# Gadersd/stable-diffusion-xl-burn

Hardware: NVIDIA H100
Metric: unet_sampler_steps_per_sec_1024x1024_bs1 (higher is better)
Workload: dtype f16

## Files before the change

stable-diffusion-xl-burn_b200/csrc/attention.cu:

```cuda
#include <stdlib.h>

#include "common.cuh"
#include "kernels.h"

namespace sdxl {

static constexpr int kTileBytes = 128 * 128;
static constexpr int kKvStages = 3;
static constexpr int kConsumerWarps = 8;
static constexpr int kAttnThreads = kConsumerWarps * 32 + 32;
static constexpr int kAttnSmem = 1024  + kTileBytes + 2 * kKvStages * kTileBytes + 256;

__device__ __forceinline__ float ex2_approx(float x) {
  float y;
  asm("ex2.approx.ftz.f32 %0, %1;" : "=f"(y) : "f"(x));
  return y;
}
__device__ __forceinline__ uint32_t pack_half2(float a, float b) {
  __half2 t = __floats2half2_rn(a, b);
  return *reinterpret_cast<uint32_t*>(&t);
}

__device__ __forceinline__ void attn_key_block(float (&o)[32], float (&m)[2], float (&l)[2], uint32_t q_addr, const uint8_t* sK,
                                               const uint8_t* sV, uint64_t* kv_full, uint64_t* kv_empty, int j, int kb, int S,
                                               float sl2e, int lane) {
  const int st = j % kKvStages;
  mbar_wait_nocall(&kv_full[st], (j / kKvStages) & 1);
  float s[64];
  wg_fence();
  const uint32_t k_addr = smem_u32(sK + st * kTileBytes);
#pragma unroll
  for (int k = 0; k < 4; ++k) wgmma_ss_n128(s, wg_desc_sw128(q_addr + 32 * k), wg_desc_sw128(k_addr + 32 * k), k);
  wg_commit();
  wg_wait<0>();
  if (kb * 128 + 128 > S) {
#pragma unroll
    for (int jj = 0; jj < 16; ++jj)
#pragma unroll
      for (int e = 0; e < 2; ++e)
        if (kb * 128 + 8 * jj + 2 * (lane & 3) + e >= S) { s[4 * jj + e] = -INFINITY; s[4 * jj + 2 + e] = -INFINITY; }
  }
  uint32_t pa[32];
#pragma unroll
  for (int h = 0; h < 2; ++h) {
    float mx = -INFINITY;
#pragma unroll
    for (int jj = 0; jj < 16; ++jj) mx = fmaxf(mx, fmaxf(s[4 * jj + 2 * h], s[4 * jj + 2 * h + 1]));
    mx = fmaxf(mx, __shfl_xor_sync(0xffffffffu, mx, 1));
    mx = fmaxf(mx, __shfl_xor_sync(0xffffffffu, mx, 2));
    const float m_new = fmaxf(m[h], mx);
    const float alpha = ex2_approx((m[h] - m_new) * sl2e);
    const float mb = m_new * sl2e;
    float sum = 0.f;
#pragma unroll
    for (int jj = 0; jj < 16; ++jj) {
      const float p0 = ex2_approx(fmaf(s[4 * jj + 2 * h], sl2e, -mb));
      const float p1 = ex2_approx(fmaf(s[4 * jj + 2 * h + 1], sl2e, -mb));
      sum += p0 + p1;
      pa[4 * (jj >> 1) + 2 * (jj & 1) + h] = pack_half2(p0, p1);
    }
    l[h] = l[h] * alpha + sum;
    m[h] = m_new;
#pragma unroll
    for (int jj = 0; jj < 8; ++jj) { o[4 * jj + 2 * h] *= alpha; o[4 * jj + 2 * h + 1] *= alpha; }
  }
  wg_fence();
  const uint32_t v_addr = smem_u32(sV + st * kTileBytes);
#pragma unroll
  for (int kk = 0; kk < 8; ++kk)
    wgmma_rs_n64_tb(o, *reinterpret_cast<const uint32_t(*)[4]>(pa + 4 * kk), wg_desc_sw128(v_addr + 2048 * kk));
  wg_commit();
  wg_wait<0>();
  if (lane == 0) mbar_arrive(&kv_empty[st]);
}

template <bool kIp>
__global__ void __launch_bounds__(kAttnThreads, 1) attention_kernel(const __grid_constant__ AttnParams p) {
  extern __shared__ uint8_t smem_raw[];
  uint8_t* smem = reinterpret_cast<uint8_t*>((reinterpret_cast<uintptr_t>(smem_raw) + 1023) & ~uintptr_t(1023));
  uint8_t* sQ = smem;
  uint8_t* sK = sQ + kTileBytes;
  uint8_t* sV = sK + kKvStages * kTileBytes;
  uint64_t* bars = reinterpret_cast<uint64_t*>(sV + kKvStages * kTileBytes);
  uint64_t* q_full = bars;
  uint64_t* kv_full = q_full + 1;
  uint64_t* kv_empty = kv_full + kKvStages;

  const int warp = threadIdx.x >> 5, lane = threadIdx.x & 31;
  const int nblk = (p.S + 127) / 128;
  const int nqt = (p.T + 127) / 128;
  const int qt = blockIdx.x % nqt, head = (blockIdx.x / nqt) % p.n_head, b = blockIdx.x / (nqt * p.n_head);

  if (threadIdx.x == 0) {
    tma_prefetch_desc(&p.tmQ);
    tma_prefetch_desc(&p.tmK);
    tma_prefetch_desc(&p.tmV);
    if constexpr (kIp) {
      tma_prefetch_desc(&p.tmKip);
      tma_prefetch_desc(&p.tmVip);
    }
    mbar_init(q_full, 1);
    for (int i = 0; i < kKvStages; ++i) { mbar_init(&kv_full[i], 1); mbar_init(&kv_empty[i], kConsumerWarps); }
    fence_barrier_init();
  }
  __syncthreads();
  griddep_wait();
  griddep_launch_dependents();

  if (warp == kConsumerWarps) {
    if (lane != 0) return;
    mbar_expect_tx(q_full, kTileBytes);
    tma_load_3d(sQ, &p.tmQ, q_full, p.q_col0 + head * 64, qt * 128, b);
    for (int j = 0; j < nblk; ++j) {
      const int st = j % kKvStages;
      mbar_wait_nocall(&kv_empty[st], ((j / kKvStages) & 1) ^ 1);
      mbar_expect_tx(&kv_full[st], 2 * kTileBytes);
      tma_load_3d(sK + st * kTileBytes, &p.tmK, &kv_full[st], p.k_col0 + head * 64, j * 128, b);
      tma_load_3d(sV + st * kTileBytes, &p.tmV, &kv_full[st], p.v_col0 + head * 64, j * 128, b);
    }
    if constexpr (kIp) {
      const int nblk_ip = (p.S_ip + 127) / 128;
      for (int j = nblk; j < nblk + nblk_ip; ++j) {
        const int st = j % kKvStages;
        mbar_wait_nocall(&kv_empty[st], ((j / kKvStages) & 1) ^ 1);
        mbar_expect_tx(&kv_full[st], 2 * kTileBytes);
        tma_load_3d(sK + st * kTileBytes, &p.tmKip, &kv_full[st], p.k_ip_col0 + head * 64, (j - nblk) * 128, b);
        tma_load_3d(sV + st * kTileBytes, &p.tmVip, &kv_full[st], p.v_ip_col0 + head * 64, (j - nblk) * 128, b);
      }
    }
    return;
  }

  const int wg = warp >> 2;
  const float sl2e = p.scale_log2e;
  const uint32_t q_addr = smem_u32(sQ) + (uint32_t)wg * (64 * 128);
  float o[32];
#pragma unroll
  for (int i = 0; i < 32; ++i) o[i] = 0.f;
  float m[2] = {-INFINITY, -INFINITY}, l[2] = {0.f, 0.f};
  mbar_wait_nocall(q_full, 0);
  for (int j = 0; j < nblk; ++j) {
    const int st = j % kKvStages;
    mbar_wait_nocall(&kv_full[st], (j / kKvStages) & 1);
    float s[64];
    wg_fence();
    const uint32_t k_addr = smem_u32(sK + st * kTileBytes);
#pragma unroll
    for (int k = 0; k < 4; ++k) wgmma_ss_n128(s, wg_desc_sw128(q_addr + 32 * k), wg_desc_sw128(k_addr + 32 * k), k);
    wg_commit();
    wg_wait<0>();
    if (j * 128 + 128 > p.S) {
#pragma unroll
      for (int jj = 0; jj < 16; ++jj)
#pragma unroll
        for (int e = 0; e < 2; ++e)
          if (j * 128 + 8 * jj + 2 * (lane & 3) + e >= p.S) { s[4 * jj + e] = -INFINITY; s[4 * jj + 2 + e] = -INFINITY; }
    }
    uint32_t pa[32];
#pragma unroll
    for (int h = 0; h < 2; ++h) {
      float mx = -INFINITY;
#pragma unroll
      for (int jj = 0; jj < 16; ++jj) mx = fmaxf(mx, fmaxf(s[4 * jj + 2 * h], s[4 * jj + 2 * h + 1]));
      mx = fmaxf(mx, __shfl_xor_sync(0xffffffffu, mx, 1));
      mx = fmaxf(mx, __shfl_xor_sync(0xffffffffu, mx, 2));
      const float m_new = fmaxf(m[h], mx);
      const float alpha = ex2_approx((m[h] - m_new) * sl2e);
      const float mb = m_new * sl2e;
      float sum = 0.f;
#pragma unroll
      for (int jj = 0; jj < 16; ++jj) {
        const float p0 = ex2_approx(fmaf(s[4 * jj + 2 * h], sl2e, -mb));
        const float p1 = ex2_approx(fmaf(s[4 * jj + 2 * h + 1], sl2e, -mb));
        sum += p0 + p1;
        pa[4 * (jj >> 1) + 2 * (jj & 1) + h] = pack_half2(p0, p1);
      }
      l[h] = l[h] * alpha + sum;
      m[h] = m_new;
#pragma unroll
      for (int jj = 0; jj < 8; ++jj) { o[4 * jj + 2 * h] *= alpha; o[4 * jj + 2 * h + 1] *= alpha; }
    }
    wg_fence();
    const uint32_t v_addr = smem_u32(sV + st * kTileBytes);
#pragma unroll
    for (int kk = 0; kk < 8; ++kk)
      wgmma_rs_n64_tb(o, *reinterpret_cast<const uint32_t(*)[4]>(pa + 4 * kk), wg_desc_sw128(v_addr + 2048 * kk));
    wg_commit();
    wg_wait<0>();
    if (lane == 0) mbar_arrive(&kv_empty[st]);
  }
  float ot[kIp ? 32 : 1];
  float s_ip = 0.f;
  if constexpr (kIp) {
#pragma unroll
    for (int h = 0; h < 2; ++h) {
      float lt = l[h];
      lt += __shfl_xor_sync(0xffffffffu, lt, 1);
      lt += __shfl_xor_sync(0xffffffffu, lt, 2);
      const float inv = 1.0f / lt;
#pragma unroll
      for (int jj = 0; jj < 8; ++jj) {
        ot[4 * jj + 2 * h] = o[4 * jj + 2 * h] * inv;
        ot[4 * jj + 2 * h + 1] = o[4 * jj + 2 * h + 1] * inv;
      }
      m[h] = -INFINITY;
      l[h] = 0.f;
    }
#pragma unroll
    for (int i = 0; i < 32; ++i) o[i] = 0.f;
    const int nblk_ip = (p.S_ip + 127) / 128;
    for (int j = nblk; j < nblk + nblk_ip; ++j) attn_key_block(o, m, l, q_addr, sK, sV, kv_full, kv_empty, j, j - nblk, p.S_ip, sl2e, lane);
    s_ip = *p.ip_scale;
  }
  const int r = wg * 64 + (warp & 3) * 16 + (lane >> 2);
#pragma unroll
  for (int h = 0; h < 2; ++h) {
    float lt = l[h];
    lt += __shfl_xor_sync(0xffffffffu, lt, 1);
    lt += __shfl_xor_sync(0xffffffffu, lt, 2);
    const float inv = 1.0f / lt;
    const int t = qt * 128 + r + 8 * h;
    if (t < p.T) {
      __half* out = p.out + ((size_t)b * p.T + t) * p.ldo + head * 64 + 2 * (lane & 3);
#pragma unroll
      for (int jj = 0; jj < 8; ++jj) {
        if constexpr (kIp)
          *reinterpret_cast<__half2*>(out + 8 * jj) = __floats2half2_rn(fmaf(s_ip, o[4 * jj + 2 * h] * inv, ot[4 * jj + 2 * h]),
                                                                        fmaf(s_ip, o[4 * jj + 2 * h + 1] * inv, ot[4 * jj + 2 * h + 1]));
        else
          *reinterpret_cast<__half2*>(out + 8 * jj) = __floats2half2_rn(o[4 * jj + 2 * h] * inv, o[4 * jj + 2 * h + 1] * inv);
      }
    }
  }
}

static bool g_attn_attr[2][64];
int attention_launch(cudaStream_t st, const AttnParams& p) {
  if (p.T < 1 || p.S < 1 || (p.ldo & 1)) return 2002;
  const bool ip = p.S_ip > 0;
  if (ip && !p.ip_scale) return 2002;
  auto kernel = ip ? attention_kernel<true> : attention_kernel<false>;
  int r = smem_optin(kernel, kAttnSmem, g_attn_attr[ip]);
  if (r) return r;
  const long tiles = (long)p.B * p.n_head * ((p.T + 127) / 128);
  return launch_kernel(kernel, dim3((unsigned)tiles), dim3(kAttnThreads), (size_t)kAttnSmem, st, true, p);
}

}
```

stable-diffusion-xl-burn_b200/csrc/common.cuh:

```cuda
#pragma once
#include <cuda_fp16.h>
#include <cuda_runtime.h>
#include <stdint.h>
#include <stdio.h>

namespace sdxl {

__device__ __forceinline__ uint32_t smem_u32(const void* p) {
  return static_cast<uint32_t>(__cvta_generic_to_shared(p));
}
__device__ __forceinline__ float warp_sum(float v) {
#pragma unroll
  for (int o = 16; o > 0; o >>= 1) v += __shfl_xor_sync(0xffffffffu, v, o);
  return v;
}
__device__ __forceinline__ float warp_max(float v) {
#pragma unroll
  for (int o = 16; o > 0; o >>= 1) v = fmaxf(v, __shfl_xor_sync(0xffffffffu, v, o));
  return v;
}
__device__ __forceinline__ float silu_f(float x) { return x / (1.0f + __expf(-x)); }
__device__ __forceinline__ float erf_as(float x) {
  const float ax = fabsf(x);
  float t;
  asm("rcp.approx.ftz.f32 %0, %1;" : "=f"(t) : "f"(fmaf(0.3275911f, ax, 1.0f)));
  const float poly =
      t * (0.254829592f + t * (-0.284496736f + t * (1.421413741f + t * (-1.453152027f + t * 1.061405429f))));
  float e;
  asm("ex2.approx.ftz.f32 %0, %1;" : "=f"(e) : "f"(-ax * ax * 1.4426950408889634f));
  return copysignf(1.0f - poly * e, x);
}
__device__ __forceinline__ float gelu_erf_f(float x) {
  return 0.5f * x * (1.0f + erf_as(x * 0.70710678118654752440f));
}
__device__ __forceinline__ uint64_t globaltimer_ns() {
  uint64_t t;
  asm volatile("mov.u64 %0, %globaltimer;" : "=l"(t)::"memory");
  return t;
}

template <int N>
__device__ __forceinline__ void setmaxnreg_dec() { asm volatile("setmaxnreg.dec.sync.aligned.u32 %0;" ::"n"(N)); }
template <int N>
__device__ __forceinline__ void setmaxnreg_inc() { asm volatile("setmaxnreg.inc.sync.aligned.u32 %0;" ::"n"(N)); }

__device__ __forceinline__ void griddep_wait() { asm volatile("griddepcontrol.wait;" ::: "memory"); }
__device__ __forceinline__ void griddep_launch_dependents() {
  asm volatile("griddepcontrol.launch_dependents;" ::: "memory");
}

__device__ __forceinline__ void mbar_init(uint64_t* bar, uint32_t count) {
  asm volatile("mbarrier.init.shared::cta.b64 [%0], %1;" ::"r"(smem_u32(bar)), "r"(count));
}
__device__ __forceinline__ void fence_barrier_init() {
  asm volatile("fence.mbarrier_init.release.cluster;" ::: "memory");
}
__device__ __forceinline__ void mbar_expect_tx(uint64_t* bar, uint32_t bytes) {
  asm volatile("mbarrier.arrive.expect_tx.shared::cta.b64 _, [%0], %1;" ::"r"(smem_u32(bar)),
               "r"(bytes)
               : "memory");
}
__device__ __forceinline__ void mbar_arrive(uint64_t* bar) {
  asm volatile("mbarrier.arrive.shared::cta.b64 _, [%0];" ::"r"(smem_u32(bar)) : "memory");
}
__device__ __forceinline__ bool mbar_try_wait(uint64_t* bar, uint32_t parity) {
  uint32_t ok;
  asm volatile(
      "{\n\t"
      ".reg .pred p;\n\t"
      "mbarrier.try_wait.parity.shared::cta.b64 p, [%1], %2;\n\t"
      "selp.u32 %0, 1, 0, p;\n\t"
      "}"
      : "=r"(ok)
      : "r"(smem_u32(bar)), "r"(parity)
      : "memory");
  return ok != 0;
}
__device__ __forceinline__ void mbar_wait(uint64_t* bar, uint32_t parity) {
  if (mbar_try_wait(bar, parity)) return;
  const uint64_t t0 = globaltimer_ns();
  while (!mbar_try_wait(bar, parity)) {
    if (globaltimer_ns() - t0 > 4000000000ull) {
      printf("sdxl_b200: mbarrier wait timeout (block %d,%d,%d thread %d)\n", blockIdx.x, blockIdx.y,
             blockIdx.z, threadIdx.x);
      __trap();
    }
  }
}
__device__ __forceinline__ void mbar_wait_nocall(uint64_t* bar, uint32_t parity) {
  if (mbar_try_wait(bar, parity)) return;
  const uint64_t t0 = globaltimer_ns();
  while (!mbar_try_wait(bar, parity))
    if (globaltimer_ns() - t0 > 4000000000ull) __trap();
}
__device__ __forceinline__ void fence_proxy_async_smem() {
  asm volatile("fence.proxy.async.shared::cta;" ::: "memory");
}

__device__ __forceinline__ void tma_prefetch_desc(const void* tmap) {
  asm volatile("prefetch.tensormap [%0];" ::"l"(reinterpret_cast<uint64_t>(tmap)) : "memory");
}
__device__ __forceinline__ void tma_load_2d(void* dst, const void* tmap, uint64_t* bar, int c0, int c1) {
  asm volatile(
      "cp.async.bulk.tensor.2d.shared::cluster.global.mbarrier::complete_tx::bytes [%0], [%1, {%3, %4}], [%2];"
      ::"r"(smem_u32(dst)), "l"(reinterpret_cast<uint64_t>(tmap)), "r"(smem_u32(bar)), "r"(c0), "r"(c1)
      : "memory");
}
__device__ __forceinline__ void tma_load_3d(void* dst, const void* tmap, uint64_t* bar, int c0, int c1,
                                            int c2) {
  asm volatile(
      "cp.async.bulk.tensor.3d.shared::cluster.global.mbarrier::complete_tx::bytes [%0], [%1, {%3, %4, %5}], [%2];"
      ::"r"(smem_u32(dst)), "l"(reinterpret_cast<uint64_t>(tmap)), "r"(smem_u32(bar)), "r"(c0), "r"(c1),
      "r"(c2)
      : "memory");
}
__device__ __forceinline__ void tma_load_4d(void* dst, const void* tmap, uint64_t* bar, int c0, int c1,
                                            int c2, int c3) {
  asm volatile(
      "cp.async.bulk.tensor.4d.shared::cluster.global.mbarrier::complete_tx::bytes [%0], [%1, {%3, %4, %5, %6}], [%2];"
      ::"r"(smem_u32(dst)), "l"(reinterpret_cast<uint64_t>(tmap)), "r"(smem_u32(bar)), "r"(c0), "r"(c1),
      "r"(c2), "r"(c3)
      : "memory");
}

__device__ __forceinline__ void wg_fence() { asm volatile("wgmma.fence.sync.aligned;" ::: "memory"); }
__device__ __forceinline__ void wg_commit() { asm volatile("wgmma.commit_group.sync.aligned;" ::: "memory"); }
template <int N>
__device__ __forceinline__ void wg_wait() {
  asm volatile("wgmma.wait_group.sync.aligned %0;" ::"n"(N) : "memory");
}
__device__ __forceinline__ uint64_t wg_desc_sw128(uint32_t saddr) {
  const uint32_t lo = ((saddr >> 4) & 0x3FFFu) | (1u << 16);
  const uint32_t hi = 64u  | (1u << 30) ;
  return (static_cast<uint64_t>(hi) << 32) | lo;
}
__device__ __forceinline__ void wgmma_ss_n160(float (&d)[80], uint64_t da, uint64_t db, int scale_d) {
  asm volatile(
      "{\n\t.reg .pred p;\n\tsetp.ne.b32 p, %82, 0;\n\t"
      "wgmma.mma_async.sync.aligned.m64n160k16.f32.f16.f16 {%0, %1, %2, %3, %4, %5, %6, %7, %8, %9, %10, %11, %12, %13, %14, %15, %16, %17, %18, %19, %20, %21, %22, %23, %24, %25, %26, %27, %28, %29, %30, %31, %32, %33, %34, %35, %36, %37, %38, %39, %40, %41, %42, %43, %44, %45, %46, %47, %48, %49, %50, %51, %52, %53, %54, %55, %56, %57, %58, %59, %60, %61, %62, %63, %64, %65, %66, %67, %68, %69, %70, %71, %72, %73, %74, %75, %76, %77, %78, %79}, %80, %81, p, 1, 1, 0, 0;\n\t}"
      : "+f"(d[0]), "+f"(d[1]), "+f"(d[2]), "+f"(d[3]), "+f"(d[4]), "+f"(d[5]), "+f"(d[6]), "+f"(d[7]), "+f"(d[8]), "+f"(d[9]), "+f"(d[10]), "+f"(d[11]), "+f"(d[12]), "+f"(d[13]), "+f"(d[14]), "+f"(d[15]), "+f"(d[16]), "+f"(d[17]), "+f"(d[18]), "+f"(d[19]), "+f"(d[20]), "+f"(d[21]), "+f"(d[22]), "+f"(d[23]), "+f"(d[24]), "+f"(d[25]), "+f"(d[26]), "+f"(d[27]), "+f"(d[28]), "+f"(d[29]), "+f"(d[30]), "+f"(d[31]), "+f"(d[32]), "+f"(d[33]), "+f"(d[34]), "+f"(d[35]), "+f"(d[36]), "+f"(d[37]), "+f"(d[38]), "+f"(d[39]), "+f"(d[40]), "+f"(d[41]), "+f"(d[42]), "+f"(d[43]), "+f"(d[44]), "+f"(d[45]), "+f"(d[46]), "+f"(d[47]), "+f"(d[48]), "+f"(d[49]), "+f"(d[50]), "+f"(d[51]), "+f"(d[52]), "+f"(d[53]), "+f"(d[54]), "+f"(d[55]), "+f"(d[56]), "+f"(d[57]), "+f"(d[58]), "+f"(d[59]), "+f"(d[60]), "+f"(d[61]), "+f"(d[62]), "+f"(d[63]), "+f"(d[64]), "+f"(d[65]), "+f"(d[66]), "+f"(d[67]), "+f"(d[68]), "+f"(d[69]), "+f"(d[70]), "+f"(d[71]), "+f"(d[72]), "+f"(d[73]), "+f"(d[74]), "+f"(d[75]), "+f"(d[76]), "+f"(d[77]), "+f"(d[78]), "+f"(d[79])
      : "l"(da), "l"(db), "r"(scale_d));
}
__device__ __forceinline__ void wgmma_ss_n128(float (&d)[64], uint64_t da, uint64_t db, int scale_d) {
  asm volatile(
      "{\n\t.reg .pred p;\n\tsetp.ne.b32 p, %66, 0;\n\t"
      "wgmma.mma_async.sync.aligned.m64n128k16.f32.f16.f16 {%0, %1, %2, %3, %4, %5, %6, %7, %8, %9, %10, %11, %12, %13, %14, %15, %16, %17, %18, %19, %20, %21, %22, %23, %24, %25, %26, %27, %28, %29, %30, %31, %32, %33, %34, %35, %36, %37, %38, %39, %40, %41, %42, %43, %44, %45, %46, %47, %48, %49, %50, %51, %52, %53, %54, %55, %56, %57, %58, %59, %60, %61, %62, %63}, %64, %65, p, 1, 1, 0, 0;\n\t}"
      : "+f"(d[0]), "+f"(d[1]), "+f"(d[2]), "+f"(d[3]), "+f"(d[4]), "+f"(d[5]), "+f"(d[6]), "+f"(d[7]), "+f"(d[8]), "+f"(d[9]), "+f"(d[10]), "+f"(d[11]), "+f"(d[12]), "+f"(d[13]), "+f"(d[14]), "+f"(d[15]), "+f"(d[16]), "+f"(d[17]), "+f"(d[18]), "+f"(d[19]), "+f"(d[20]), "+f"(d[21]), "+f"(d[22]), "+f"(d[23]), "+f"(d[24]), "+f"(d[25]), "+f"(d[26]), "+f"(d[27]), "+f"(d[28]), "+f"(d[29]), "+f"(d[30]), "+f"(d[31]), "+f"(d[32]), "+f"(d[33]), "+f"(d[34]), "+f"(d[35]), "+f"(d[36]), "+f"(d[37]), "+f"(d[38]), "+f"(d[39]), "+f"(d[40]), "+f"(d[41]), "+f"(d[42]), "+f"(d[43]), "+f"(d[44]), "+f"(d[45]), "+f"(d[46]), "+f"(d[47]), "+f"(d[48]), "+f"(d[49]), "+f"(d[50]), "+f"(d[51]), "+f"(d[52]), "+f"(d[53]), "+f"(d[54]), "+f"(d[55]), "+f"(d[56]), "+f"(d[57]), "+f"(d[58]), "+f"(d[59]), "+f"(d[60]), "+f"(d[61]), "+f"(d[62]), "+f"(d[63])
      : "l"(da), "l"(db), "r"(scale_d));
}
__device__ __forceinline__ void wgmma_ss_n64(float (&d)[32], uint64_t da, uint64_t db, int scale_d) {
  asm volatile(
      "{\n\t.reg .pred p;\n\tsetp.ne.b32 p, %34, 0;\n\t"
      "wgmma.mma_async.sync.aligned.m64n64k16.f32.f16.f16 {%0, %1, %2, %3, %4, %5, %6, %7, %8, %9, %10, %11, %12, %13, %14, %15, %16, %17, %18, %19, %20, %21, %22, %23, %24, %25, %26, %27, %28, %29, %30, %31}, %32, %33, p, 1, 1, 0, 0;\n\t}"
      : "+f"(d[0]), "+f"(d[1]), "+f"(d[2]), "+f"(d[3]), "+f"(d[4]), "+f"(d[5]), "+f"(d[6]), "+f"(d[7]), "+f"(d[8]), "+f"(d[9]), "+f"(d[10]), "+f"(d[11]), "+f"(d[12]), "+f"(d[13]), "+f"(d[14]), "+f"(d[15]), "+f"(d[16]), "+f"(d[17]), "+f"(d[18]), "+f"(d[19]), "+f"(d[20]), "+f"(d[21]), "+f"(d[22]), "+f"(d[23]), "+f"(d[24]), "+f"(d[25]), "+f"(d[26]), "+f"(d[27]), "+f"(d[28]), "+f"(d[29]), "+f"(d[30]), "+f"(d[31])
      : "l"(da), "l"(db), "r"(scale_d));
}
__device__ __forceinline__ void wgmma_rs_n64_tb(float (&d)[32], const uint32_t (&a)[4], uint64_t db) {
  asm volatile(
      "{\n\t.reg .pred p;\n\tsetp.eq.b32 p, 0, 0;\n\t"
      "wgmma.mma_async.sync.aligned.m64n64k16.f32.f16.f16 {%0, %1, %2, %3, %4, %5, %6, %7, %8, %9, %10, %11, %12, %13, %14, %15, %16, %17, %18, %19, %20, %21, %22, %23, %24, %25, %26, %27, %28, %29, %30, %31}, {%32, %33, %34, %35}, %36, p, 1, 1, 1;\n\t}"
      : "+f"(d[0]), "+f"(d[1]), "+f"(d[2]), "+f"(d[3]), "+f"(d[4]), "+f"(d[5]), "+f"(d[6]), "+f"(d[7]), "+f"(d[8]), "+f"(d[9]), "+f"(d[10]), "+f"(d[11]), "+f"(d[12]), "+f"(d[13]), "+f"(d[14]), "+f"(d[15]), "+f"(d[16]), "+f"(d[17]), "+f"(d[18]), "+f"(d[19]), "+f"(d[20]), "+f"(d[21]), "+f"(d[22]), "+f"(d[23]), "+f"(d[24]), "+f"(d[25]), "+f"(d[26]), "+f"(d[27]), "+f"(d[28]), "+f"(d[29]), "+f"(d[30]), "+f"(d[31])
      : "r"(a[0]), "r"(a[1]), "r"(a[2]), "r"(a[3]), "l"(db));
}

}
```

Baseline: 21.61.

## Pipeline QK and PV wgmma with ping-pong warpgroup scheduling in attention

Restructures the attention consumer loop so the QK^T MMA for the next key block is issued together with the PV MMA of the previous block. Softmax of the current block then runs while the PV MMA is still in flight. Named barriers make the two consumer warpgroups alternate MMA issue in ping-pong fashion, so one warpgroup's softmax overlaps the other's tensor-core work. It also raises the KV pipeline depth from 3 to 4 stages and moves the IP-adapter intermediate output into shared memory to relieve register pressure. The cost is more shared memory, extra barrier synchronisation, and some risk of register spills or ordering bugs.

```diff
diff --git a/stable-diffusion-xl-burn_b200/csrc/attention.cu b/stable-diffusion-xl-burn_b200/csrc/attention.cu
--- a/stable-diffusion-xl-burn_b200/csrc/attention.cu
+++ b/stable-diffusion-xl-burn_b200/csrc/attention.cu
@@ -6,10 +6,11 @@
 namespace sdxl {
 
 static constexpr int kTileBytes = 128 * 128;
-static constexpr int kKvStages = 3;
+static constexpr int kKvStages = 4;
 static constexpr int kConsumerWarps = 8;
 static constexpr int kAttnThreads = kConsumerWarps * 32 + 32;
 static constexpr int kAttnSmem = 1024  + kTileBytes + 2 * kKvStages * kTileBytes + 256;
+static constexpr int kAttnSmemIp = kAttnSmem + 32 * kConsumerWarps * 32 * 4;
 
 __device__ __forceinline__ float ex2_approx(float x) {
   float y;
@@ -21,18 +22,27 @@
   return *reinterpret_cast<uint32_t*>(&t);
 }
 
-__device__ __forceinline__ void attn_key_block(float (&o)[32], float (&m)[2], float (&l)[2], uint32_t q_addr, const uint8_t* sK,
-                                               const uint8_t* sV, uint64_t* kv_full, uint64_t* kv_empty, int j, int kb, int S,
-                                               float sl2e, int lane) {
+__device__ __forceinline__ void issue_qk(float (&s)[64], uint32_t q_addr, const uint8_t* sK, uint64_t* kv_full, int j) {
   const int st = j % kKvStages;
   mbar_wait_nocall(&kv_full[st], (j / kKvStages) & 1);
-  float s[64];
   wg_fence();
   const uint32_t k_addr = smem_u32(sK + st * kTileBytes);
 #pragma unroll
   for (int k = 0; k < 4; ++k) wgmma_ss_n128(s, wg_desc_sw128(q_addr + 32 * k), wg_desc_sw128(k_addr + 32 * k), k);
   wg_commit();
-  wg_wait<0>();
+}
+
+__device__ __forceinline__ void issue_pv(float (&o)[32], const uint32_t (&pa)[32], const uint8_t* sV, int j) {
+  wg_fence();
+  const uint32_t v_addr = smem_u32(sV + (j % kKvStages) * kTileBytes);
+#pragma unroll
+  for (int kk = 0; kk < 8; ++kk)
+    wgmma_rs_n64_tb(o, *reinterpret_cast<const uint32_t(*)[4]>(pa + 4 * kk), wg_desc_sw128(v_addr + 2048 * kk));
+  wg_commit();
+}
+
+__device__ __forceinline__ void softmax_block(float (&s)[64], float (&m)[2], float (&l)[2], float (&alpha)[2], int kb, int S,
+                                              float sl2e, int lane) {
   if (kb * 128 + 128 > S) {
 #pragma unroll
     for (int jj = 0; jj < 16; ++jj)
@@ -40,7 +50,6 @@
       for (int e = 0; e < 2; ++e)
         if (kb * 128 + 8 * jj + 2 * (lane & 3) + e >= S) { s[4 * jj + e] = -INFINITY; s[4 * jj + 2 + e] = -INFINITY; }
   }
-  uint32_t pa[32];
 #pragma unroll
   for (int h = 0; h < 2; ++h) {
     float mx = -INFINITY;
@@ -49,29 +58,64 @@
     mx = fmaxf(mx, __shfl_xor_sync(0xffffffffu, mx, 1));
     mx = fmaxf(mx, __shfl_xor_sync(0xffffffffu, mx, 2));
     const float m_new = fmaxf(m[h], mx);
-    const float alpha = ex2_approx((m[h] - m_new) * sl2e);
+    alpha[h] = ex2_approx((m[h] - m_new) * sl2e);
     const float mb = m_new * sl2e;
     float sum = 0.f;
 #pragma unroll
     for (int jj = 0; jj < 16; ++jj) {
-      const float p0 = ex2_approx(fmaf(s[4 * jj + 2 * h], sl2e, -mb));
-      const float p1 = ex2_approx(fmaf(s[4 * jj + 2 * h + 1], sl2e, -mb));
-      sum += p0 + p1;
-      pa[4 * (jj >> 1) + 2 * (jj & 1) + h] = pack_half2(p0, p1);
-    }
-    l[h] = l[h] * alpha + sum;
+      s[4 * jj + 2 * h] = ex2_approx(fmaf(s[4 * jj + 2 * h], sl2e, -mb));
+      s[4 * jj + 2 * h + 1] = ex2_approx(fmaf(s[4 * jj + 2 * h + 1], sl2e, -mb));
+      sum += s[4 * jj + 2 * h] + s[4 * jj + 2 * h + 1];
+    }
+    l[h] = l[h] * alpha[h] + sum;
     m[h] = m_new;
-#pragma unroll
-    for (int jj = 0; jj < 8; ++jj) { o[4 * jj + 2 * h] *= alpha; o[4 * jj + 2 * h + 1] *= alpha; }
-  }
-  wg_fence();
-  const uint32_t v_addr = smem_u32(sV + st * kTileBytes);
-#pragma unroll
-  for (int kk = 0; kk < 8; ++kk)
-    wgmma_rs_n64_tb(o, *reinterpret_cast<const uint32_t(*)[4]>(pa + 4 * kk), wg_desc_sw128(v_addr + 2048 * kk));
-  wg_commit();
+  }
+}
+
+__device__ __forceinline__ void rescale_pack(const float (&s)[64], const float (&alpha)[2], float (&o)[32], uint32_t (&pa)[32]) {
+#pragma unroll
+  for (int h = 0; h < 2; ++h) {
+#pragma unroll
+    for (int jj = 0; jj < 8; ++jj) { o[4 * jj + 2 * h] *= alpha[h]; o[4 * jj + 2 * h + 1] *= alpha[h]; }
+#pragma unroll
+    for (int jj = 0; jj < 16; ++jj) pa[4 * (jj >> 1) + 2 * (jj & 1) + h] = pack_half2(s[4 * jj + 2 * h], s[4 * jj + 2 * h + 1]);
+  }
+}
+
+__device__ __forceinline__ void turn_begin(int wg) { named_bar_sync(1 + wg, 256); }
+__device__ __forceinline__ void turn_end(int wg) { named_bar_arrive(2 - wg, 256); }
+
+__device__ __forceinline__ void attn_source(float (&o)[32], float (&m)[2], float (&l)[2], uint32_t q_addr, const uint8_t* sK,
+                                            const uint8_t* sV, uint64_t* kv_full, uint64_t* kv_empty, int j0, int n, int S,
+                                            float sl2e, int wg, int lane) {
+  float s[64], alpha[2];
+  uint32_t pa[32];
+  turn_begin(wg);
+  issue_qk(s, q_addr, sK, kv_full, j0);
+  turn_end(wg);
   wg_wait<0>();
-  if (lane == 0) mbar_arrive(&kv_empty[st]);
+  wg_fence_regs(s);
+  softmax_block(s, m, l, alpha, 0, S, sl2e, lane);
+  rescale_pack(s, alpha, o, pa);
+  for (int i = 1; i < n; ++i) {
+    turn_begin(wg);
+    issue_qk(s, q_addr, sK, kv_full, j0 + i);
+    issue_pv(o, pa, sV, j0 + i - 1);
+    turn_end(wg);
+    wg_wait<1>();
+    wg_fence_regs(s);
+    softmax_block(s, m, l, alpha, i, S, sl2e, lane);
+    wg_wait<0>();
+    wg_fence_regs(o);
+    if (lane == 0) mbar_arrive(&kv_empty[(j0 + i - 1) % kKvStages]);
+    rescale_pack(s, alpha, o, pa);
+  }
+  turn_begin(wg);
+  issue_pv(o, pa, sV, j0 + n - 1);
+  turn_end(wg);
+  wg_wait<0>();
+  wg_fence_regs(o);
+  if (lane == 0) mbar_arrive(&kv_empty[(j0 + n - 1) % kKvStages]);
 }
 
 template <bool kIp>
@@ -85,6 +129,7 @@
   uint64_t* q_full = bars;
   uint64_t* kv_full = q_full + 1;
   uint64_t* kv_empty = kv_full + kKvStages;
+  float* s_ot = reinterpret_cast<float*>(bars + 32);
 
   const int warp = threadIdx.x >> 5, lane = threadIdx.x & 31;
   const int nblk = (p.S + 127) / 128;
@@ -138,58 +183,9 @@
 #pragma unroll
   for (int i = 0; i < 32; ++i) o[i] = 0.f;
   float m[2] = {-INFINITY, -INFINITY}, l[2] = {0.f, 0.f};
+  if (wg == 1) turn_end(wg);
   mbar_wait_nocall(q_full, 0);
-  for (int j = 0; j < nblk; ++j) {
-    const int st = j % kKvStages;
-    mbar_wait_nocall(&kv_full[st], (j / kKvStages) & 1);
-    float s[64];
-    wg_fence();
-    const uint32_t k_addr = smem_u32(sK + st * kTileBytes);
-#pragma unroll
-    for (int k = 0; k < 4; ++k) wgmma_ss_n128(s, wg_desc_sw128(q_addr + 32 * k), wg_desc_sw128(k_addr + 32 * k), k);
-    wg_commit();
-    wg_wait<0>();
-    if (j * 128 + 128 > p.S) {
-#pragma unroll
-      for (int jj = 0; jj < 16; ++jj)
-#pragma unroll
-        for (int e = 0; e < 2; ++e)
-          if (j * 128 + 8 * jj + 2 * (lane & 3) + e >= p.S) { s[4 * jj + e] = -INFINITY; s[4 * jj + 2 + e] = -INFINITY; }
-    }
-    uint32_t pa[32];
-#pragma unroll
-    for (int h = 0; h < 2; ++h) {
-      float mx = -INFINITY;
-#pragma unroll
-      for (int jj = 0; jj < 16; ++jj) mx = fmaxf(mx, fmaxf(s[4 * jj + 2 * h], s[4 * jj + 2 * h + 1]));
-      mx = fmaxf(mx, __shfl_xor_sync(0xffffffffu, mx, 1));
-      mx = fmaxf(mx, __shfl_xor_sync(0xffffffffu, mx, 2));
-      const float m_new = fmaxf(m[h], mx);
-      const float alpha = ex2_approx((m[h] - m_new) * sl2e);
-      const float mb = m_new * sl2e;
-      float sum = 0.f;
-#pragma unroll
-      for (int jj = 0; jj < 16; ++jj) {
-        const float p0 = ex2_approx(fmaf(s[4 * jj + 2 * h], sl2e, -mb));
-        const float p1 = ex2_approx(fmaf(s[4 * jj + 2 * h + 1], sl2e, -mb));
-        sum += p0 + p1;
-        pa[4 * (jj >> 1) + 2 * (jj & 1) + h] = pack_half2(p0, p1);
-      }
-      l[h] = l[h] * alpha + sum;
-      m[h] = m_new;
-#pragma unroll
-      for (int jj = 0; jj < 8; ++jj) { o[4 * jj + 2 * h] *= alpha; o[4 * jj + 2 * h + 1] *= alpha; }
-    }
-    wg_fence();
-    const uint32_t v_addr = smem_u32(sV + st * kTileBytes);
-#pragma unroll
-    for (int kk = 0; kk < 8; ++kk)
-      wgmma_rs_n64_tb(o, *reinterpret_cast<const uint32_t(*)[4]>(pa + 4 * kk), wg_desc_sw128(v_addr + 2048 * kk));
-    wg_commit();
-    wg_wait<0>();
-    if (lane == 0) mbar_arrive(&kv_empty[st]);
-  }
-  float ot[kIp ? 32 : 1];
+  attn_source(o, m, l, q_addr, sK, sV, kv_full, kv_empty, 0, nblk, p.S, sl2e, wg, lane);
   float s_ip = 0.f;
   if constexpr (kIp) {
 #pragma unroll
@@ -200,18 +196,18 @@
       const float inv = 1.0f / lt;
 #pragma unroll
       for (int jj = 0; jj < 8; ++jj) {
-        ot[4 * jj + 2 * h] = o[4 * jj + 2 * h] * inv;
-        ot[4 * jj + 2 * h + 1] = o[4 * jj + 2 * h + 1] * inv;
+        s_ot[(4 * jj + 2 * h) * (kConsumerWarps * 32) + threadIdx.x] = o[4 * jj + 2 * h] * inv;
+        s_ot[(4 * jj + 2 * h + 1) * (kConsumerWarps * 32) + threadIdx.x] = o[4 * jj + 2 * h + 1] * inv;
       }
       m[h] = -INFINITY;
       l[h] = 0.f;
     }
 #pragma unroll
     for (int i = 0; i < 32; ++i) o[i] = 0.f;
-    const int nblk_ip = (p.S_ip + 127) / 128;
-    for (int j = nblk; j < nblk + nblk_ip; ++j) attn_key_block(o, m, l, q_addr, sK, sV, kv_full, kv_empty, j, j - nblk, p.S_ip, sl2e, lane);
+    attn_source(o, m, l, q_addr, sK, sV, kv_full, kv_empty, nblk, (p.S_ip + 127) / 128, p.S_ip, sl2e, wg, lane);
     s_ip = *p.ip_scale;
   }
+  if (wg == 0) turn_begin(wg);
   const int r = wg * 64 + (warp & 3) * 16 + (lane >> 2);
 #pragma unroll
   for (int h = 0; h < 2; ++h) {
@@ -225,8 +221,8 @@
 #pragma unroll
       for (int jj = 0; jj < 8; ++jj) {
         if constexpr (kIp)
-          *reinterpret_cast<__half2*>(out + 8 * jj) = __floats2half2_rn(fmaf(s_ip, o[4 * jj + 2 * h] * inv, ot[4 * jj + 2 * h]),
-                                                                        fmaf(s_ip, o[4 * jj + 2 * h + 1] * inv, ot[4 * jj + 2 * h + 1]));
+          *reinterpret_cast<__half2*>(out + 8 * jj) = __floats2half2_rn(fmaf(s_ip, o[4 * jj + 2 * h] * inv, s_ot[(4 * jj + 2 * h) * (kConsumerWarps * 32) + threadIdx.x]),
+                                                                        fmaf(s_ip, o[4 * jj + 2 * h + 1] * inv, s_ot[(4 * jj + 2 * h + 1) * (kConsumerWarps * 32) + threadIdx.x]));
         else
           *reinterpret_cast<__half2*>(out + 8 * jj) = __floats2half2_rn(o[4 * jj + 2 * h] * inv, o[4 * jj + 2 * h + 1] * inv);
       }
@@ -240,10 +236,11 @@
   const bool ip = p.S_ip > 0;
   if (ip && !p.ip_scale) return 2002;
   auto kernel = ip ? attention_kernel<true> : attention_kernel<false>;
-  int r = smem_optin(kernel, kAttnSmem, g_attn_attr[ip]);
+  const int smem = ip ? kAttnSmemIp : kAttnSmem;
+  int r = smem_optin(kernel, smem, g_attn_attr[ip]);
   if (r) return r;
   const long tiles = (long)p.B * p.n_head * ((p.T + 127) / 128);
-  return launch_kernel(kernel, dim3((unsigned)tiles), dim3(kAttnThreads), (size_t)kAttnSmem, st, true, p);
-}
-
-}
+  return launch_kernel(kernel, dim3((unsigned)tiles), dim3(kAttnThreads), (size_t)smem, st, true, p);
+}
+
+}
diff --git a/stable-diffusion-xl-burn_b200/csrc/common.cuh b/stable-diffusion-xl-burn_b200/csrc/common.cuh
--- a/stable-diffusion-xl-burn_b200/csrc/common.cuh
+++ b/stable-diffusion-xl-burn_b200/csrc/common.cuh
@@ -43,6 +43,13 @@
 __device__ __forceinline__ void setmaxnreg_dec() { asm volatile("setmaxnreg.dec.sync.aligned.u32 %0;" ::"n"(N)); }
 template <int N>
 __device__ __forceinline__ void setmaxnreg_inc() { asm volatile("setmaxnreg.inc.sync.aligned.u32 %0;" ::"n"(N)); }
+
+__device__ __forceinline__ void named_bar_sync(int id, int count) {
+  asm volatile("bar.sync %0, %1;" ::"r"(id), "r"(count) : "memory");
+}
+__device__ __forceinline__ void named_bar_arrive(int id, int count) {
+  asm volatile("bar.arrive %0, %1;" ::"r"(id), "r"(count) : "memory");
+}
 
 __device__ __forceinline__ void griddep_wait() { asm volatile("griddepcontrol.wait;" ::: "memory"); }
 __device__ __forceinline__ void griddep_launch_dependents() {
@@ -129,6 +136,11 @@
 __device__ __forceinline__ void wg_wait() {
   asm volatile("wgmma.wait_group.sync.aligned %0;" ::"n"(N) : "memory");
 }
+template <int N>
+__device__ __forceinline__ void wg_fence_regs(float (&r)[N]) {
+#pragma unroll
+  for (int i = 0; i < N; ++i) asm volatile("" : "+f"(r[i]));
+}
 __device__ __forceinline__ uint64_t wg_desc_sw128(uint32_t saddr) {
   const uint32_t lo = ((saddr >> 4) & 0x3FFFu) | (1u << 16);
   const uint32_t hi = 64u  | (1u << 30) ;
```

Result: faster. 21.82, median of 6 (+1.0%).
